# Tarekbouamer/Image-Retrieval-for-Image-Based-Localization

Measured on AMD Instinct MI355X. Metric: images/sec extract + queries/sec 1M-desc kNN, ResNet50-GeM 1024×768, higher is better.
Workload: dtype fp16

## Files before the change

image-retrieval-for-image-based-localization_amd/csrc/rr_c3pair.hip:

```cpp
#include "rr_internal.h"

#ifndef C3P_IG2
#define C3P_IG2 1
#endif

namespace rr {

namespace {

typedef __attribute__((ext_vector_type(4))) float cf32x4_t;
typedef __attribute__((ext_vector_type(4))) int ci32x4_t;

constexpr unsigned COOB = 0x80000000u;

__device__ __forceinline__ void cdma16(ci32x4_t rsrc, unsigned voff, unsigned lds_addr) {
    unsigned keep;
    lds_addr = __builtin_amdgcn_readfirstlane(lds_addr);
    asm volatile(
        "s_mov_b32 %0, m0\n\t"
        "s_mov_b32 m0, %3\n\t"
        "s_nop 0\n\t"
        "buffer_load_dwordx4 %1, %2, 0 offen lds\n\t"
        "s_mov_b32 m0, %0"
        : "=&s"(keep)
        : "v"(voff), "s"(rsrc), "s"(lds_addr)
        : "memory");
}

__device__ __forceinline__ ci32x4_t crsrc(const void* base, unsigned bytes) {
    const unsigned long long b = (unsigned long long)base;
    ci32x4_t r;
    r.x = __builtin_amdgcn_readfirstlane((int)(unsigned)b);
    r.y = __builtin_amdgcn_readfirstlane((int)((unsigned)(b >> 32) & 0xFFFFu));
    r.z = __builtin_amdgcn_readfirstlane((int)bytes);
    r.w = 0x00020000;
    int x = r.x, y = r.y, z = r.z;
    asm volatile("s_nop 4" : "+s"(x), "+s"(y), "+s"(z));
    r.x = x;
    r.y = y;
    r.z = z;
    return r;
}

__device__ __forceinline__ void cbar() { asm volatile("s_waitcnt lgkmcnt(0)\n\ts_barrier" ::: "memory"); }

template <int K>
__device__ __forceinline__ int cwswz(int row, int chunk) {
    const int f = K == 64 ? ((row >> 1) & 7) : (row & 15);
    return row * (K * 2) + ((chunk ^ f) << 4);
}

__device__ __forceinline__ void cpin(uint4& v) { asm volatile("" : "+v"(v.x), "+v"(v.y), "+v"(v.z), "+v"(v.w)); }

}

struct C3PairArgs {
    const bf16_t* t1;
    const bf16_t* w0;
    const float *s0, *h0;
    const bf16_t* w33;
    const float *s33, *h33;
    const bf16_t* w3;
    const float *s3, *h3;
    const bf16_t* res;
    const bf16_t* xp;
    const bf16_t* wp;
    const float *sp, *hp;
    const bf16_t* w1;
    const float *s1, *h1;
    bf16_t* y;
    bf16_t* z;
    int* queue;
    int n, h, w;
    int act2, act3, act1, act0;
    float slope2, slope3, slope1, slope0;
};

namespace {

template <int C1, bool PROJ, typename HT, bool CONV1 = false>
__global__ void __launch_bounds__(512, 1) k_c3pair(C3PairArgs a, int tiles_w, int tiles_hw, int ntiles) {
    static_assert(!CONV1 || PROJ, "conv1 in the launch: the stage's first block only");
    constexpr int TH = 4, TW = 32, TP = TH * TW, PITCH = 40;
    constexpr int NSLOT = (TH + 2) * PITCH, NP = NSLOT / 8;
    constexpr int PCW = TW + 2;
    constexpr int FN = 4;
    constexpr int K3 = 64, C3 = 256, NK3 = K3 / 32, NR3 = C3 / 32, NF1 = C1 / 16, NK1 = C3 / 32;
    static_assert(NSLOT % 8 == 0 && PITCH % 8 == 0, "row-invariant patch swizzle");
    __shared__ __attribute__((aligned(1024))) char sPatch[NSLOT * 128];
    __shared__ __attribute__((aligned(16))) char sT2[TP * 128];
    __shared__ __attribute__((aligned(16))) char sW3[C3 * K3 * 2];
    __shared__ __attribute__((aligned(16))) char sW1[C1 * C3 * 2];
    __shared__ __attribute__((aligned(16))) char sWp[PROJ ? C3 * K3 * 2 : 16];
    __shared__ __attribute__((aligned(16))) float sS3[C3], sH3[C3], sS1[C1], sH1[C1], sS2[64], sH2[64];
    __shared__ __attribute__((aligned(16))) float sSp[PROJ ? C3 : 4], sHp[PROJ ? C3 : 4];
    __shared__ __attribute__((aligned(16))) char sW0[CONV1 ? 64 * 64 * 2 : 16];
    __shared__ __attribute__((aligned(16))) float sS0[CONV1 ? 64 : 4], sH0[CONV1 ? 64 : 4];
    __shared__ int sTile[4];

    const int tid = threadIdx.x, lane = tid & 63;
    const int wave = __builtin_amdgcn_readfirstlane(tid >> 6);
    const bool role3 = wave < 4;
    const int r16 = lane & 15, kq = lane >> 4, lrow = lane >> 3, lch = lane & 7;
    const int H = a.h, W = a.w;

    for (int i = tid; i < C3 * K3 / 8; i += 512) {
        const int r = i / (K3 / 8), c = i - r * (K3 / 8);
        *reinterpret_cast<uint4*>(sW3 + cwswz<K3>(r, c)) = reinterpret_cast<const uint4*>(a.w3)[i];
        if constexpr (PROJ) *reinterpret_cast<uint4*>(sWp + cwswz<K3>(r, c)) = reinterpret_cast<const uint4*>(a.wp)[i];
    }
    for (int i = tid; i < C1 * C3 / 8; i += 512) {
        const int r = i / (C3 / 8), c = i - r * (C3 / 8);
        *reinterpret_cast<uint4*>(sW1 + cwswz<C3>(r, c)) = reinterpret_cast<const uint4*>(a.w1)[i];
    }
    for (int i = tid; i < C3; i += 512) {
        sS3[i] = a.s3[i];
        sH3[i] = a.h3[i];
        if constexpr (PROJ) {
            sSp[i] = a.sp[i];
            sHp[i] = a.hp[i];
        }
    }
    for (int i = tid; i < C1; i += 512) {
        sS1[i] = a.s1[i];
        sH1[i] = a.h1[i];
    }
    if (tid < 64) {
        sS2[tid] = a.s33[tid];
        sH2[tid] = a.h33[tid];
        if constexpr (CONV1) {
            sS0[tid] = a.s0[tid];
            sH0[tid] = a.h0[tid];
        }
    }
    if constexpr (CONV1)
        for (int i = tid; i < 64 * 64 / 8; i += 512) {
            const int r = i / 8, c = i - r * 8;
            *reinterpret_cast<uint4*>(sW0 + cwswz<64>(r, c)) = reinterpret_cast<const uint4*>(a.w0)[i];
        }
    const int wc = wave & 1, wpx = (wave >> 1) & 1;

    const int b = (int)blockIdx.x, G = (int)gridDim.x, xcd = b & 7;
    const int nt8 = ntiles >> 3, rt8 = ntiles & 7;
    const int s_x = xcd < rt8 ? xcd * (nt8 + 1) : rt8 * (nt8 + 1) + (xcd - rt8) * nt8;
    const int n_x = nt8 + (xcd < rt8 ? 1 : 0);
    auto fetch_tile = [&](int i) __attribute__((always_inline)) {
        if (a.queue) {
            const int v = atomicAdd(a.queue + xcd, 1);
            return v < n_x ? s_x + v : -1;
        }
        const int t = i * G + xcd * (G >> 3) + (b >> 3);
        return t < ntiles ? t : -1;
    };
    if (tid == 0) {
        sTile[0] = fetch_tile(0);
        sTile[1] = fetch_tile(1);
        sTile[2] = fetch_tile(2);
    }
    __syncthreads();
    auto tile_id = [&](int i) __attribute__((always_inline)) { return sTile[i & 3]; };
    if (tile_id(0) < 0) return;
    auto tile_org = [&](int t, int& img, int& oh0, int& ow0) __attribute__((always_inline)) {
        img = t / tiles_hw;
        const int rem = t - img * tiles_hw, th = rem / tiles_w;
        oh0 = th * TH;
        ow0 = (rem - th * tiles_w) * TW;
    };

    const ci32x4_t rsX = crsrc(a.t1, (unsigned)((long long)a.n * H * W * 64 * 2));
    const unsigned ldsP = (unsigned)(unsigned long long)sPatch;
    auto patch_dma = [&](int t, bool live) __attribute__((always_inline)) {
        int img = 0, oh0 = 0, ow0 = 0;
        if (live) tile_org(t, img, oh0, ow0);
        int lr = lrow;
        asm volatile("" : "+v"(lr));
#pragma unroll
        for (int u = 0; u < 8; ++u) {
            const int d = wave + 4 * u, q = d * 8 + lr;
            if (d >= NP) break;
            const int pr = q / PITCH, pc = q - pr * PITCH;
            const int hh = oh0 - 1 + pr, ww = ow0 - 1 + pc;
            unsigned off = COOB;
            if (live && pc < PCW && (unsigned)hh < (unsigned)H && (unsigned)ww < (unsigned)W)
                off = (unsigned)(((((long long)img * H + hh) * W + ww) * 64 + ((lch ^ lr) << 3)) * 2);
            cdma16(rsX, off, ldsP + d * 1024);
        }
    };
    h16_f32x4_t acc[2][FN];
    auto conv3x3 = [&](const uint4 (&areg)[2][18]) __attribute__((always_inline)) {
        int lc;
        asm volatile("v_mbcnt_lo_u32_b32 %0, -1, 0\n\tv_mbcnt_hi_u32_b32 %0, -1, %0" : "=v"(lc));
        lc &= 15;
        const char* base[FN][3][2];
#pragma unroll
        for (int j = 0; j < FN; ++j)
#pragma unroll
            for (int dx = 0; dx < 3; ++dx)
#pragma unroll
                for (int hs = 0; hs < 2; ++hs) {
                    const int q = (wpx * 2 + (j >> 1)) * PITCH + (j & 1) * 16 + lc + dx;
                    base[j][dx][hs] = sPatch + q * 128 + (((kq + 4 * hs) ^ (q & 7)) << 4);
                }
#pragma unroll
        for (int ii = 0; ii < 2; ++ii)
#pragma unroll
            for (int j = 0; j < FN; ++j) acc[ii][j] = (h16_f32x4_t){0.f, 0.f, 0.f, 0.f};
#pragma unroll
        for (int s = 0; s < 18; ++s) {
            const int tap = s >> 1, hs = s & 1, dy = tap / 3, dx = tap % 3;
            uint4 fb[FN];
#pragma unroll
            for (int j = 0; j < FN; ++j) fb[j] = *reinterpret_cast<const uint4*>(base[j][dx][hs] + dy * PITCH * 128);
#pragma unroll
            for (int ii = 0; ii < 2; ++ii)
#pragma unroll
                for (int j = 0; j < FN; ++j) acc[ii][j] = H16<HT>::mfma(areg[ii][s], fb[j], acc[ii][j]);
        }
    };
    auto convert_patch = [&](int t) __attribute__((always_inline)) {
        if constexpr (CONV1) {
            int img, oh0, ow0;
            tile_org(t, img, oh0, ow0);
            const bool leaky0 = a.act0 == RR_ACT_LEAKY;
            for (int f = wave; f < NP * 8 / 16; f += 4) {
                int q = f * 16 + r16;
                asm volatile("" : "+v"(q));
                const int pr = q / PITCH, pc = q - pr * PITCH;
                const int hh = oh0 - 1 + pr, ww = ow0 - 1 + pc;
                const bool valid = pc < PCW && (unsigned)hh < (unsigned)H && (unsigned)ww < (unsigned)W;
                char* slot = sPatch + q * 128;
                uint4 bx[2];
#pragma unroll
                for (int kk = 0; kk < 2; ++kk)
                    bx[kk] = *reinterpret_cast<const uint4*>(slot + (((4 * kk + kq) ^ (q & 7)) << 4));
                h16_f32x4_t c0[4];
#pragma unroll
                for (int ii = 0; ii < 4; ++ii) c0[ii] = (h16_f32x4_t){0.f, 0.f, 0.f, 0.f};
#pragma unroll
                for (int kk = 0; kk < 2; ++kk)
#pragma unroll
                    for (int ii = 0; ii < 4; ++ii) {
                        const uint4 av = *reinterpret_cast<const uint4*>(sW0 + cwswz<64>(ii * 16 + r16, kk * 4 + kq));
                        c0[ii] = H16<HT>::mfma(av, bx[kk], c0[ii]);
                    }
#pragma unroll
                for (int i2 = 0; i2 < 2; ++i2) {
                    const int c = 32 * i2 + 8 * kq;
                    float v[8];
#pragma unroll
                    for (int r = 0; r < 4; ++r) {
                        v[r] = c0[2 * i2][r] * sS0[c + r] + sH0[c + r];
                        v[4 + r] = c0[2 * i2 + 1][r] * sS0[c + 4 + r] + sH0[c + 4 + r];
                    }
                    if (leaky0) {
#pragma unroll
                        for (int r = 0; r < 8; ++r) v[r] = v[r] > 0.f ? v[r] : v[r] * a.slope0;
                    }
                    uint4 o = make_uint4(0u, 0u, 0u, 0u);
                    if (valid) {
                        o.x = H16<HT>::pack2(v[0], v[1]);
                        o.y = H16<HT>::pack2(v[2], v[3]);
                        o.z = H16<HT>::pack2(v[4], v[5]);
                        o.w = H16<HT>::pack2(v[6], v[7]);
                    }
                    *reinterpret_cast<uint4*>(slot + (((4 * i2 + kq) ^ (q & 7)) << 4)) = o;
                }
            }
        }
    };
    auto store_t2 = [&]() __attribute__((always_inline)) {
        const int c = 32 * wc + 8 * kq;
        float sc[8], sh[8];
#pragma unroll
        for (int r = 0; r < 8; ++r) {
            sc[r] = sS2[c + r];
            sh[r] = sH2[c + r];
        }
        const bool leaky2 = a.act2 == RR_ACT_LEAKY;
#pragma unroll
        for (int j = 0; j < FN; ++j) {
            const int p = wpx * (TP / 2) + j * 16 + r16;
            float v[8];
#pragma unroll
            for (int r = 0; r < 4; ++r) {
                v[r] = acc[0][j][r] * sc[r] + sh[r];
                v[4 + r] = acc[1][j][r] * sc[4 + r] + sh[4 + r];
            }
            if (leaky2) {
#pragma unroll
                for (int r = 0; r < 8; ++r) v[r] = v[r] > 0.f ? v[r] : v[r] * a.slope2;
            }
            uint4 o;
            o.x = H16<HT>::pack2(v[0], v[1]);
            o.y = H16<HT>::pack2(v[2], v[3]);
            o.z = H16<HT>::pack2(v[4], v[5]);
            o.w = H16<HT>::pack2(v[6], v[7]);
            *reinterpret_cast<uint4*>(sT2 + p * 128 + (((4 * wc + kq) ^ (p & 7)) << 4)) = o;
        }
    };

    const int pw = wave - 4;
    const bool leaky3 = a.act3 == RR_ACT_LEAKY, leaky1 = a.act1 == RR_ACT_LEAKY;
    constexpr int NRQ = PROJ ? NK3 : NR3;
    auto strip_pixel = [&](int t, int k) __attribute__((always_inline)) {
        int img, oh0, ow0;
        tile_org(t, img, oh0, ow0);
        return ((long long)img * H + oh0 + (k >> 1)) * W + ow0 + (k & 1) * 16 + r16;
    };
    auto load_rq = [&](uint4 (&dst)[NRQ], long long p) __attribute__((always_inline)) {
        if constexpr (PROJ) {
            const bf16_t* ps = a.xp + p * K3 + 8 * kq;
#pragma unroll
            for (int kk = 0; kk < NK3; ++kk) dst[kk] = ld16_once(ps + kk * 32);
        } else {
            const bf16_t* rs = a.res + p * C3 + 8 * kq;
#pragma unroll
            for (int i2 = 0; i2 < NR3; ++i2) dst[i2] = ld16_once(rs + 32 * i2);
        }
    };
    auto pair_strip = [&](int k, long long p, const uint4 (&rv)[NRQ]) __attribute__((always_inline)) {
        uint4 bq[NK3];
        {
            const int q = k * 16 + r16;
#pragma unroll
            for (int kk = 0; kk < NK3; ++kk)
                bq[kk] = *reinterpret_cast<const uint4*>(sT2 + q * 128 + (((4 * kk + kq) ^ (q & 7)) << 4));
        }
        uint4 yq[NR3];
        constexpr int IG = C3P_IG2 ? 2 : 1;
#pragma unroll
        for (int i0 = 0; i0 < NR3; i0 += IG) {
            int abase = 0;
            asm volatile("" : "+v"(abase));
            h16_f32x4_t acc3[IG][2], pacc[IG][2];
#pragma unroll
            for (int g = 0; g < IG; ++g)
#pragma unroll
                for (int hh = 0; hh < 2; ++hh) acc3[g][hh] = pacc[g][hh] = (h16_f32x4_t){0.f, 0.f, 0.f, 0.f};
#pragma unroll
            for (int kk = 0; kk < NK3; ++kk)
#pragma unroll
                for (int g = 0; g < IG; ++g)
#pragma unroll
                    for (int hh = 0; hh < 2; ++hh) {
                        const uint4 av = *reinterpret_cast<const uint4*>(sW3 + abase + cwswz<K3>((2 * (i0 + g) + hh) * 16 + r16, kk * 4 + kq));
                        acc3[g][hh] = H16<HT>::mfma(av, bq[kk], acc3[g][hh]);
                    }
            if constexpr (PROJ) {
#pragma unroll
                for (int kk = 0; kk < NK3; ++kk)
#pragma unroll
                    for (int g = 0; g < IG; ++g)
#pragma unroll
                        for (int hh = 0; hh < 2; ++hh) {
                            const uint4 av = *reinterpret_cast<const uint4*>(sWp + abase + cwswz<K3>((2 * (i0 + g) + hh) * 16 + r16, kk * 4 + kq));
                            pacc[g][hh] = H16<HT>::mfma(av, rv[kk], pacc[g][hh]);
                        }
            }
#pragma unroll
            for (int g = 0; g < IG; ++g) {
                const int i2 = i0 + g;
                const int c = 32 * i2 + 8 * kq;
                float v[8];
#pragma unroll
                for (int r = 0; r < 4; ++r) {
                    v[r] = acc3[g][0][r] * sS3[c + r] + sH3[c + r];
                    v[4 + r] = acc3[g][1][r] * sS3[c + 4 + r] + sH3[c + 4 + r];
                }
                if constexpr (PROJ) {
#pragma unroll
                    for (int r = 0; r < 4; ++r) {
                        v[r] += pacc[g][0][r] * sSp[c + r] + sHp[c + r];
                        v[4 + r] += pacc[g][1][r] * sSp[c + 4 + r] + sHp[c + 4 + r];
                    }
                } else {
                    const uint4 qv = rv[i2];
                    const unsigned w4[4] = {qv.x, qv.y, qv.z, qv.w};
#pragma unroll
                    for (int r = 0; r < 4; ++r) {
                        v[2 * r] += H16<HT>::lo(w4[r]);
                        v[2 * r + 1] += H16<HT>::hi(w4[r]);
                    }
                }
                if (leaky3) {
#pragma unroll
                    for (int r = 0; r < 8; ++r) v[r] = v[r] > 0.f ? v[r] : v[r] * a.slope3;
                }
                yq[i2].x = H16<HT>::pack2(v[0], v[1]);
                yq[i2].y = H16<HT>::pack2(v[2], v[3]);
                yq[i2].z = H16<HT>::pack2(v[4], v[5]);
                yq[i2].w = H16<HT>::pack2(v[6], v[7]);
                st16_once(a.y + p * C3 + c, yq[i2]);
            }
        }
        h16_f32x4_t zacc[NF1];
#pragma unroll
        for (int o = 0; o < NF1; ++o) zacc[o] = (h16_f32x4_t){0.f, 0.f, 0.f, 0.f};
#pragma unroll
        for (int kk = 0; kk < NK1; ++kk) {
            int abase = 0;
            asm volatile("" : "+v"(abase));
#pragma unroll
            for (int o = 0; o < NF1; ++o) {
                const uint4 av = *reinterpret_cast<const uint4*>(sW1 + abase + cwswz<C3>(o * 16 + r16, kk * 4 + kq));
                zacc[o] = H16<HT>::mfma(av, yq[kk], zacc[o]);
            }
        }
#pragma unroll
        for (int o2 = 0; o2 < NF1 / 2; ++o2) {
            const int c = 32 * o2 + 8 * kq;
            float v[8];
#pragma unroll
            for (int r = 0; r < 4; ++r) {
                v[r] = zacc[2 * o2][r] * sS1[c + r] + sH1[c + r];
                v[4 + r] = zacc[2 * o2 + 1][r] * sS1[c + 4 + r] + sH1[c + 4 + r];
            }
            if (leaky1) {
#pragma unroll
                for (int r = 0; r < 8; ++r) v[r] = v[r] > 0.f ? v[r] : v[r] * a.slope1;
            }
            uint4 o;
            o.x = H16<HT>::pack2(v[0], v[1]);
            o.y = H16<HT>::pack2(v[2], v[3]);
            o.z = H16<HT>::pack2(v[4], v[5]);
            o.w = H16<HT>::pack2(v[6], v[7]);
            st16_once(a.z + p * C1 + c, o);
        }
    };

    if (role3) {
        uint4 areg[2][18];
#pragma unroll
        for (int i = 0; i < 2; ++i)
#pragma unroll
            for (int ks = 0; ks < 18; ++ks)
                areg[i][ks] = *reinterpret_cast<const uint4*>(a.w33 + (long long)(32 * wc + 16 * i + r16) * 576 +
                                                              (ks >> 1) * 64 + 32 * (ks & 1) + 8 * kq);
#pragma unroll
        for (int i = 0; i < 2; ++i)
#pragma unroll
            for (int ks = 0; ks < 18; ++ks) cpin(areg[i][ks]);
        auto conv = [&]() __attribute__((always_inline)) { conv3x3(areg); };
        patch_dma(tile_id(0), true);
        asm volatile("s_waitcnt vmcnt(0)" ::: "memory");
        cbar();
        if constexpr (CONV1) {
            convert_patch(tile_id(0));
            cbar();
        }
        conv();
        if (wpx == 0) store_t2();
        cbar();
        patch_dma(tile_id(1), tile_id(1) >= 0);
        asm volatile("s_waitcnt vmcnt(0)" ::: "memory");
        cbar();
        for (int s = 0; tile_id(s) >= 0; ++s) {
            const bool more = tile_id(s + 1) >= 0;
            if (wpx == 1) store_t2();
            if constexpr (CONV1) {
                if (more) convert_patch(tile_id(s + 1));
                cbar();
            }
            if (more) conv();
            cbar();
            if (more) {
                if (wpx == 0) store_t2();
                const int t2i = tile_id(s + 2);
                patch_dma(t2i, t2i >= 0);
                if (tid == 0) sTile[(s + 3) & 3] = t2i >= 0 ? fetch_tile(s + 3) : -1;
                asm volatile("s_waitcnt vmcnt(0)" ::: "memory");
            }
            cbar();
        }
    } else {
        __builtin_amdgcn_s_setprio(1);
        uint4 rq[4][NRQ];
        load_rq(rq[0], strip_pixel(tile_id(0), pw));
        load_rq(rq[1], strip_pixel(tile_id(0), 4 + pw));
        cbar();
        if constexpr (CONV1) cbar();
        cbar();
        cbar();
        for (int s = 0; tile_id(s) >= 0; s += 2) {
            {
                const int t = tile_id(s);
                const bool n1 = tile_id(s + 1) >= 0;
                if (n1) load_rq(rq[2], strip_pixel(tile_id(s + 1), pw));
                if constexpr (CONV1) cbar();
                pair_strip(pw, strip_pixel(t, pw), rq[0]);
                cbar();
                if (n1) load_rq(rq[3], strip_pixel(tile_id(s + 1), 4 + pw));
                pair_strip(4 + pw, strip_pixel(t, 4 + pw), rq[1]);
                cbar();
            }
            if (tile_id(s + 1) >= 0) {
                const int t = tile_id(s + 1);
                const bool n2 = tile_id(s + 2) >= 0;
                if (n2) load_rq(rq[0], strip_pixel(tile_id(s + 2), pw));
                if constexpr (CONV1) cbar();
                pair_strip(pw, strip_pixel(t, pw), rq[2]);
                cbar();
                if (n2) load_rq(rq[1], strip_pixel(tile_id(s + 2), 4 + pw));
                pair_strip(4 + pw, strip_pixel(t, 4 + pw), rq[3]);
                cbar();
            }
        }
    }
}

}

}

using namespace rr;

extern "C" int rr_conv3x3_pair(const void* t1, int n, int h, int w, const void* w0, const float* scale0,
                               const float* shift0, int act0, float slope0, const void* w33, const float* scale2,
                               const float* shift2, int act2, float slope2, const void* w3, const float* scale3,
                               const float* shift3, const void* residual, const void* xp, const void* wp,
                               const float* scalep, const float* shiftp, int act3, float slope3, const void* w1,
                               const float* scale1, const float* shift1, int c_out, int act1, float slope1, void* y,
                               void* z, int* tile_queue, int dtype, void* stream) {
    if (dtype != RR_BF16 && dtype != RR_F16) return fail(RR_EINVAL, "rr_conv3x3_pair: dtype (bf16 / fp16)");
    if (!t1 || !w33 || !scale2 || !shift2 || !w3 || !scale3 || !shift3 || !w1 || !scale1 || !shift1 || !y || !z)
        return fail(RR_EINVAL, "rr_conv3x3_pair: null pointer");
    const bool proj = residual == nullptr;
    if (proj && (!xp || !wp || !scalep || !shiftp))
        return fail(RR_EINVAL, "rr_conv3x3_pair: either residual or the projection (xp, wp, scalep, shiftp)");
    if (c_out != 64 && c_out != 128) return fail(RR_EINVAL, "rr_conv3x3_pair: c_out 64 or 128");
    if (proj && c_out != 64) return fail(RR_EINVAL, "rr_conv3x3_pair: the projection form takes c_out = 64");
    const bool conv1 = w0 != nullptr;
    if (conv1 && (!proj || !scale0 || !shift0 || ((uintptr_t)w0 & 15)))
        return fail(RR_EINVAL, "rr_conv3x3_pair: conv1 in the launch (w0) needs the projection form, scale0, shift0");
    if (conv1 && act0 != RR_ACT_IDENTITY && act0 != RR_ACT_LEAKY) return fail(RR_EINVAL, "rr_conv3x3_pair: act0");
    if (n <= 0 || h <= 0 || w <= 0 || h % 4 || w % 32) return fail(RR_EINVAL, "rr_conv3x3_pair: h % 4, w % 32");
    if ((long long)n * h * w * 64 * 2 >= (1ll << 31)) return fail(RR_EINVAL, "rr_conv3x3_pair: t1 over 2 GiB (split the batch)");
    for (const void* p : {t1, w33, w3, residual, xp, wp, w1, (const void*)y, (const void*)z})
        if ((uintptr_t)p & 15) return fail(RR_EINVAL, "rr_conv3x3_pair: 16-byte alignment required");
    if ((uintptr_t)tile_queue & 3) return fail(RR_EINVAL, "rr_conv3x3_pair: tile_queue alignment");
    for (int act : {act2, act3, act1})
        if (act != RR_ACT_IDENTITY && act != RR_ACT_LEAKY) return fail(RR_EINVAL, "rr_conv3x3_pair: activation");
    C3PairArgs a;
    a.t1 = (const bf16_t*)t1; a.w33 = (const bf16_t*)w33; a.s33 = scale2; a.h33 = shift2;
    a.w3 = (const bf16_t*)w3; a.s3 = scale3; a.h3 = shift3; a.res = (const bf16_t*)residual;
    a.xp = (const bf16_t*)xp; a.wp = (const bf16_t*)wp; a.sp = scalep; a.hp = shiftp;
    a.w1 = (const bf16_t*)w1; a.s1 = scale1; a.h1 = shift1; a.y = (bf16_t*)y; a.z = (bf16_t*)z;
    a.n = n; a.h = h; a.w = w; a.act2 = act2; a.act3 = act3; a.act1 = act1;
    a.slope2 = slope2; a.slope3 = slope3; a.slope1 = slope1; a.queue = tile_queue;
    a.w0 = (const bf16_t*)w0; a.s0 = scale0; a.h0 = shift0; a.act0 = act0; a.slope0 = slope0;
    const int tiles_w = w / 32, tiles_hw = (h / 4) * tiles_w;
    const long long ntl = (long long)n * tiles_hw;
    if (ntl >= (1ll << 31)) return fail(RR_EINVAL, "rr_conv3x3_pair: too many tiles");
    const int cus = grid_cus();
    int grid = (int)(ntl < cus ? ntl : cus) & ~7;
    if (grid < 8) grid = 8;
    const dim3 g((unsigned)grid), b(512);
    hipStream_t s = as_stream(stream);
    auto go = [&](auto hv) {
        using H = decltype(hv);
        if (conv1) hipLaunchKernelGGL((k_c3pair<64, true, H, true>), g, b, 0, s, a, tiles_w, tiles_hw, (int)ntl);
        else if (proj) hipLaunchKernelGGL((k_c3pair<64, true, H>), g, b, 0, s, a, tiles_w, tiles_hw, (int)ntl);
        else if (c_out == 64) hipLaunchKernelGGL((k_c3pair<64, false, H>), g, b, 0, s, a, tiles_w, tiles_hw, (int)ntl);
        else hipLaunchKernelGGL((k_c3pair<128, false, H>), g, b, 0, s, a, tiles_w, tiles_hw, (int)ntl);
    };
    if (dtype == RR_F16) go(f16_t{});
    else go(bf16_t{});
    return check_launch("rr_conv3x3_pair");
}
```

image-retrieval-for-image-based-localization_amd/csrc/rr_stream.hip:

```cpp
#include "rr_internal.h"

namespace rr {

namespace {

typedef __attribute__((ext_vector_type(4))) float sf32x4_t;

template <int K>
__device__ __forceinline__ int wswz(int row, int chunk) {
    const int f = K == 64 ? ((row >> 1) & 7) : (row & 15);
    return row * (K * 2) + ((chunk ^ f) << 4);
}

template <int TC, int K, int FN, int D, int NW, bool RES, typename H>
__global__ void __launch_bounds__(64 * NW) k_stream1x1(ConvArgs a, int nslices, int xmap) {
    constexpr int NI = TC / 16;
    constexpr int NK = K / 32;
    constexpr int NR = TC / 32;
    constexpr int SP = 16 * FN;
    constexpr bool AREG = NI * NK * 4 <= 32;
    __shared__ __attribute__((aligned(16))) char sA[TC * K * 2];
    __shared__ __attribute__((aligned(16))) float sS[TC], sH[TC];

    const int tid = threadIdx.x, lane = tid & 63;
// ... 741 lines not shown
template <int K, int CW, bool RES, typename H, bool DEEP = true>
__global__ void __launch_bounds__(512, 1) k_wres1x1(WresArgs a) {
    constexpr int TP = 32, NJ = TP / 16, NI = CW / 16, NK = K / 32, BC = 8 * CW;
    constexpr int XRB = K * 2, RRB = RES ? BC * 2 : 0;
    constexpr int XB = TP * XRB, RB = TP * RRB;
    constexpr int BUF = XB + RB, NBUF = RES || !DEEP ? 3 : (BUF <= 16384 ? 6 : 4), DA = NBUF - 1;
    constexpr int NDX = XB / 1024 / 8, NDR = RB / 1024 / 8;
    constexpr int ND = NDX + NDR, NST = (CW / 32) * NJ;
    static_assert(NI * NK <= 32 && XB % 8192 == 0 && RB % 8192 == 0, "tile shape");
    static_assert(XRB <= 1024 && RRB <= 1024, "row fits one DMA instruction");
    __shared__ __attribute__((aligned(1024))) char smem[NBUF * BUF];
    __shared__ __attribute__((aligned(16))) float sS[BC], sH[BC];

    const int tid = threadIdx.x, lane = tid & 63;
    const int wave = __builtin_amdgcn_readfirstlane(tid >> 6);
    const int r16 = lane & 15, kq = lane >> 4;
    const int b = (int)blockIdx.x, ns = a.nslices;
    const int slice = a.xmap ? (b >> 3) % ns : b % ns;
    const int bi = a.xmap ? ((b >> 3) / ns) * 8 + (b & 7) : b / ns;
    const int G = (int)gridDim.x / ns;
    const int c0 = slice * BC, cw0 = c0 + CW * wave;

    const bool affine = a.scale != nullptr;
    for (int i = tid; i < BC; i += 512) {
        sS[i] = affine ? a.scale[c0 + i] : 1.f;
        sH[i] = affine ? a.shift[c0 + i] : 0.f;
    }
    uint4 areg[NI][NK];
#pragma unroll
    for (int i = 0; i < NI; ++i)
#pragma unroll
        for (int kk = 0; kk < NK; ++kk)
            areg[i][kk] = *reinterpret_cast<const uint4*>(a.w + (long long)(cw0 + 16 * i + r16) * K + 32 * kk + 8 * kq);
#pragma unroll
    for (int i = 0; i < NI; ++i)
#pragma unroll
        for (int kk = 0; kk < NK; ++kk) pin_loaded(areg[i][kk]);
    __syncthreads();

    const long long P = a.P;
    const int ntiles = (int)((P + TP - 1) / TP);
    if (bi >= ntiles) return;
    const long long nimg = P / ((long long)a.ho * a.wo);
    const si32x4_t rsX = srsrc(a.x, (unsigned)(nimg * a.h * a.w_ * XRB));
    si32x4_t rsR = rsX;
    if constexpr (RES) rsR = srsrc(a.res + c0, (unsigned)(P * a.ldy * 2 - (long long)c0 * 2));
    const unsigned lds0 = (unsigned)(unsigned long long)smem;
    const int hw = a.ho * a.wo;
    auto x_row = [&](unsigned p) -> unsigned {
        if (a.stride == 1) return p;
        const unsigned img = p / (unsigned)hw, rem = p - img * (unsigned)hw;
        const unsigned oh = rem / (unsigned)a.wo, ow = rem - oh * (unsigned)a.wo;
        return (img * (unsigned)a.h + oh * (unsigned)a.stride) * (unsigned)a.w_ + ow * (unsigned)a.stride;
    };
    auto dma = [&](int t, int buf) {
#pragma unroll
        for (int u = 0; u < NDX; ++u) {
            constexpr int CPR = XRB / 16;
            const int d = NDX * wave + u, px = d * (1024 / XRB) + lane / CPR, slot = lane % CPR;
            const unsigned off = x_row((unsigned)(t * TP + px)) * XRB + (unsigned)((slot ^ (px & 15)) << 4);
            sdma16(rsX, off, lds0 + buf * BUF + d * 1024);
        }
        if constexpr (RES) {
#pragma unroll
            for (int u = 0; u < NDR; ++u) {
                constexpr int CPR = RRB / 16;
                const int d = NDR * wave + u, px = d * (1024 / RRB) + lane / CPR, slot = lane % CPR;
                const unsigned off = (unsigned)(((long long)t * TP + px) * a.ldy * 2) + (unsigned)((slot ^ (px & 15)) << 4);
                sdma16(rsR, off, lds0 + buf * BUF + XB + d * 1024);
            }
        }
    };
    const bool leaky = a.act == RR_ACT_LEAKY;

    if constexpr (DA == 2) {
        dma(bi, 0);
        if (bi + G < ntiles) dma(bi + G, 1);
    } else {
#pragma unroll
        for (int j = 0; j < DA; ++j) dma(bi + j * G, j);
    }
    for (int k = 0, t = bi; t < ntiles; ++k, t += G) {
        const int cur = k % NBUF;
        if constexpr (DA == 2) {
            if (t + G < ntiles) {
                if (k == 0) asm volatile("s_waitcnt vmcnt(%0)\n\ts_barrier" ::"n"(ND) : "memory");
                else asm volatile("s_waitcnt vmcnt(%0)\n\ts_barrier" ::"n"(ND + NST) : "memory");
            } else {
                if (k == 0) asm volatile("s_waitcnt vmcnt(0)\n\ts_barrier" ::: "memory");
                else asm volatile("s_waitcnt vmcnt(%0)\n\ts_barrier" ::"n"(NST) : "memory");
            }
            if (t + 2 * G < ntiles) dma(t + 2 * G, (k + 2) % NBUF);
        } else {
            if (k == 0) asm volatile("s_waitcnt vmcnt(%0)\n\ts_barrier" ::"n"((DA - 1) * ND) : "memory");
            else asm volatile("s_waitcnt vmcnt(%0)\n\ts_barrier" ::"n"((DA - 1) * ND + NST) : "memory");
            dma(t + DA * G, (k + DA) % NBUF);
        }
        const char* X = smem + cur * BUF;
        const char* Rt = X + XB;
        h16_f32x4_t acc[NI][NJ];
#pragma unroll
        for (int i = 0; i < NI; ++i)
#pragma unroll
            for (int j = 0; j < NJ; ++j) acc[i][j] = (h16_f32x4_t){0.f, 0.f, 0.f, 0.f};
#pragma unroll
        for (int kk = 0; kk < NK; ++kk) {
            uint4 bx[NJ];
#pragma unroll
            for (int j = 0; j < NJ; ++j) {
                const int px = 16 * j + r16;
                bx[j] = *reinterpret_cast<const uint4*>(X + px * XRB + (((4 * kk + kq) ^ (px & 15)) << 4));
            }
#pragma unroll
            for (int i = 0; i < NI; ++i)
#pragma unroll
                for (int j = 0; j < NJ; ++j) acc[i][j] = H16<H>::mfma(areg[i][kk], bx[j], acc[i][j]);
        }
#pragma unroll
        for (int i2 = 0; i2 < CW / 32; ++i2) {
            const int cl = CW * wave + 32 * i2 + 8 * kq;
            const float4 sc0 = *reinterpret_cast<const float4*>(sS + cl);
            const float4 sc1 = *reinterpret_cast<const float4*>(sS + cl + 4);
            const float4 sh0 = *reinterpret_cast<const float4*>(sH + cl);
            const float4 sh1 = *reinterpret_cast<const float4*>(sH + cl + 4);
            const float sc[8] = {sc0.x, sc0.y, sc0.z, sc0.w, sc1.x, sc1.y, sc1.z, sc1.w};
            const float sh[8] = {sh0.x, sh0.y, sh0.z, sh0.w, sh1.x, sh1.y, sh1.z, sh1.w};
#pragma unroll
            for (int j = 0; j < NJ; ++j) {
                const int px = 16 * j + r16;
                float v[8];
#pragma unroll
                for (int r = 0; r < 4; ++r) {
                    v[r] = acc[2 * i2][j][r] * sc[r] + sh[r];
                    v[4 + r] = acc[2 * i2 + 1][j][r] * sc[4 + r] + sh[4 + r];
                }
                if constexpr (RES) {
                    const uint4 q = *reinterpret_cast<const uint4*>(Rt + px * RRB + (((cl >> 3) ^ (px & 15)) << 4));
                    const unsigned w4[4] = {q.x, q.y, q.z, q.w};
#pragma unroll
                    for (int r = 0; r < 4; ++r) {
                        v[2 * r] += H16<H>::lo(w4[r]);
                        v[2 * r + 1] += H16<H>::hi(w4[r]);
                    }
                }
                if (leaky) {
#pragma unroll
                    for (int r = 0; r < 8; ++r) v[r] = v[r] > 0.f ? v[r] : v[r] * a.slope;
                }
                uint4 o;
                o.x = H16<H>::pack2(v[0], v[1]);
                o.y = H16<H>::pack2(v[2], v[3]);
                o.z = H16<H>::pack2(v[4], v[5]);
                o.w = H16<H>::pack2(v[6], v[7]);
                const long long p = (long long)t * TP + px;
                if (p < P) st16_once(a.y + p * a.ldy + c0 + cl, o);
            }
        }
    }
    asm volatile("s_waitcnt vmcnt(0)" ::: "memory");
}


template <int TC, int K, int FN, int D, int NW, typename H>
void launch_s_t(const ConvArgs& a, hipStream_t s) {
    const int g_stream_cus = grid_cus();
    constexpr int LDS = TC * K * 2 + TC * 8;
    constexpr int PER_CU = (160 * 1024 / LDS) >= 2 && NW <= 8 ? (NW <= 4 ? 4 : 2) : 1;
    const int nslices = a.cout / TC;
    const long long nstrips = ((long long)a.P + 16 * FN - 1) / (16 * FN);
    long long per_slice = (long long)PER_CU * g_stream_cus / nslices;
    if (per_slice < 1) per_slice = 1;
    const long long need = (nstrips + NW - 1) / NW;
    if (per_slice > need) per_slice = need;
    const int grid = (int)(per_slice * nslices);
    const int xmap = g_tune.stream_xcd && nslices > 1 && grid % (8 * nslices) == 0;
    if (a.flags & RR_CONV_RESIDUAL)
        hipLaunchKernelGGL((k_stream1x1<TC, K, FN, D, NW, true, H>), dim3(grid), dim3(64 * NW), 0, s, a, nslices, xmap);
    else
        hipLaunchKernelGGL((k_stream1x1<TC, K, FN, D, NW, false, H>), dim3(grid), dim3(64 * NW), 0, s, a, nslices, xmap);
}

template <int K, int CW>
void launch_wres(const ConvArgs& a, hipStream_t s, bool f16) {
    constexpr int BC = 8 * CW;
    const bool res = a.flags & RR_CONV_RESIDUAL;
    WresArgs w;
    w.w = (const bf16_t*)a.w;
    const bool affine = a.flags & RR_CONV_AFFINE;
    w.scale = affine ? a.scale : nullptr;
    w.shift = affine ? a.shift : nullptr;
    w.ldy = a.ldy;
    w.act = a.act;
    w.slope = a.slope;
    w.h = a.h; w.w_ = a.w_; w.ho = a.ho; w.wo = a.wo; w.stride = a.stride;
    w.nslices = a.cout / BC;
    int per = grid_cus() / w.nslices;
    if (per < 1) per = 1;
    const long long in_img = (long long)a.h * a.w_ * K * 2, out_img = (long long)a.ho * a.wo * a.ldy * 2;
    long long ich = (1ll << 31) / (in_img > out_img ? in_img : out_img);
    if (ich < 1) ich = 1;
    const long long hw = (long long)a.ho * a.wo;
    for (long long i0 = 0; i0 < a.n; i0 += ich) {
        const long long ni = a.n - i0 < ich ? a.n - i0 : ich;
        w.x = (const bf16_t*)a.x + i0 * a.h * a.w_ * K;
        w.res = res ? (const bf16_t*)a.res + i0 * hw * a.ldy : nullptr;
        w.y = (bf16_t*)a.y + i0 * hw * a.ldy;
        w.P = ni * hw;
        const long long ntiles = (w.P + 31) / 32;
        const int ps = (int)(per < ntiles ? per : ntiles);
        const int grid = ps * w.nslices;
        w.xmap = w.nslices > 1 && grid % (8 * w.nslices) == 0;
        auto go = [&](auto h) {
            using H = decltype(h);
            if (res) hipLaunchKernelGGL((k_wres1x1<K, CW, true, H>), dim3(grid), dim3(512), 0, s, w);
            else if (g_tune.wres_ring) hipLaunchKernelGGL((k_wres1x1<K, CW, false, H>), dim3(grid), dim3(512), 0, s, w);
            else hipLaunchKernelGGL((k_wres1x1<K, CW, false, H, false>), dim3(grid), dim3(512), 0, s, w);
        };
        if (f16) go(f16_t{});
        else go(bf16_t{});
    }
}
}

template <int TC, int K, int FN, int D, int NW>
void launch_s(const ConvArgs& a, hipStream_t s, bool f16) {
    if (f16) launch_s_t<TC, K, FN, D, NW, f16_t>(a, s);
    else launch_s_t<TC, K, FN, D, NW, bf16_t>(a, s);
}

bool gemm8_eligible(const ConvArgs& a, bool k1, int esz);

bool launch_stream1x1(const ConvArgs& a, hipStream_t s, bool f16) {
    if (g_tune.stream_1x1 == 0) return false;
    if (!(a.flags & RR_CONV_PERM32) || a.kh != 1 || a.kw != 1 || a.pad != 0 || a.kp != a.cin) return false;
    if (a.P < 4096 || (long long)a.n * a.h * a.w_ * a.cin >= (1ll << 31)) return false;
    const bool res = a.flags & RR_CONV_RESIDUAL;
    const int K = a.cin, C = a.cout;
    if (g_tune.wres && (a.ldy & 7) == 0 && (a.stride == 1 ? a.h == a.ho && a.w_ == a.wo : !res)) {
        if (K == 512 && C == 2048 && res) { launch_wres<512, 32>(a, s, f16); return true; }
        if (K == 256 && C == 1024 && res) { launch_wres<256, 64>(a, s, f16); return true; }
        if (K == 128 && C == 512 && res) { launch_wres<128, 64>(a, s, f16); return true; }
        if (g_tune.wres >= 2) {
            if (K == 512 && (C == 256 || C == 1024 || C == 2048) && !res) { launch_wres<512, 32>(a, s, f16); return true; }
            if (K == 256 && (C == 512 || C == 1024) && !res) { launch_wres<256, 64>(a, s, f16); return true; }
        }
    }
    if (g_tune.stream_1x1 >= 2 && K == 512 && C == 2048 && res && gemm8_eligible(a, true, 2)) return false;
    if (g_tune.stream_1x1 >= 3 && K == 256 && C == 1024 && res && gemm8_eligible(a, true, 2)) return false;
    if (K == 64 && C == 64) { launch_s<64, 64, 2, 4, 8>(a, s, f16); return true; }
    if (K == 64 && C == 256) { launch_s<256, 64, 1, 2, 8>(a, s, f16); return true; }
    if (K == 256 && C == 64) { launch_s<64, 256, 1, 4, 8>(a, s, f16); return true; }
    if (K == 256 && C == 128) { launch_s<128, 256, 1, 3, 8>(a, s, f16); return true; }
    if (K == 128 && C == 512) { launch_s<256, 128, 1, 3, 8>(a, s, f16); return true; }
    if (K == 512 && C == 128) { launch_s<128, 512, 1, 2, 8>(a, s, f16); return true; }
    if (K == 256 && C == 1024 && res) { launch_s<256, 256, 1, 2, 8>(a, s, f16); return true; }
    if (K == 256 && C == 512 && !res) { launch_s<256, 256, 1, 2, 8>(a, s, f16); return true; }
    if (K == 512 && C == 2048 && res) { launch_s<128, 512, 1, 2, 8>(a, s, f16); return true; }
    if (K == 512 && !res && (C == 256 || C == 1024) && gemm8_eligible(a, true, 2)) return false;
    if (K == 512 && C == 256 && !res) { launch_s<128, 512, 1, 2, 8>(a, s, f16); return true; }
    if (K == 512 && C == 1024 && !res) { launch_s<128, 512, 1, 2, 8>(a, s, f16); return true; }
    return false;
}


}

using namespace rr;

extern "C" int rr_conv1x1_pair(const void* x, long long p, int c_in, const void* w3, const float* scale3,
                               const float* shift3, int c_mid, const void* residual, const void* xp, const void* wp,
                               const float* scalep, const float* shiftp, int act3, float slope3, const void* w1,
                               const float* scale1, const float* shift1, int c_out, int act1, float slope1, void* y,
                               void* z, int dtype, void* stream) {
    if (dtype != RR_BF16 && dtype != RR_F16) return fail(RR_EINVAL, "rr_conv1x1_pair: bf16 / fp16 only");
    const bool stage2 = c_in == 64 && c_mid == 256 && (c_out == 64 || c_out == 128);
    const bool stage3 = c_in == 128 && c_mid == 512 && c_out == 128;
    if (!stage2 && !stage3)
        return fail(RR_EINVAL, "rr_conv1x1_pair: shapes (c_in 64, c_mid 256, c_out 64|128) or (128, 512, 128) only");
    if (!x || !w3 || !scale3 || !shift3 || !w1 || !scale1 || !shift1 || !y || !z)
        return fail(RR_EINVAL, "rr_conv1x1_pair: null pointer");
    const bool proj = residual == nullptr;
    if (proj && stage3) return fail(RR_EINVAL, "rr_conv1x1_pair: the 128/512 boundary needs a residual");
    if (proj && (!xp || !wp || !scalep || !shiftp))
        return fail(RR_EINVAL, "rr_conv1x1_pair: either residual or the projection (xp, wp, scalep, shiftp) is required");
    if (proj && ((((uintptr_t)xp) | ((uintptr_t)wp)) & 15))
        return fail(RR_EINVAL, "rr_conv1x1_pair: 16-byte alignment required");
    if (p <= 0) return fail(RR_EINVAL, "rr_conv1x1_pair: empty");
    if ((((uintptr_t)x) | ((uintptr_t)residual) | ((uintptr_t)y) | ((uintptr_t)z) | ((uintptr_t)w3) |
         ((uintptr_t)w1)) & 15)
        return fail(RR_EINVAL, "rr_conv1x1_pair: 16-byte alignment required");
    if (act3 != RR_ACT_IDENTITY && act3 != RR_ACT_LEAKY) return fail(RR_EINVAL, "rr_conv1x1_pair: act3");
    if (act1 != RR_ACT_IDENTITY && act1 != RR_ACT_LEAKY) return fail(RR_EINVAL, "rr_conv1x1_pair: act1");
    const int g_pair_cus = grid_cus();
    hipStream_t s = as_stream(stream);
    if (stage3) {
        constexpr long long CH = 1ll << 20;
        for (long long p0 = 0; p0 < p; p0 += CH) {
            PairMidArgs m;
            const long long pn = p - p0 < CH ? p - p0 : CH;
            m.x = (const bf16_t*)x + p0 * 128; m.w3 = (const bf16_t*)w3; m.s3 = scale3; m.h3 = shift3;
            m.res = (const bf16_t*)residual + p0 * 512; m.w1 = (const bf16_t*)w1; m.s1 = scale1; m.h1 = shift1;
            m.y = (bf16_t*)y + p0 * 512; m.z = (bf16_t*)z + p0 * 128; m.P = pn;
            m.act3 = act3; m.act1 = act1; m.slope3 = slope3; m.slope1 = slope1;
            const long long ntiles = (pn + (g_tune.pair_mid ? 31 : 63)) / (g_tune.pair_mid ? 32 : 64);
            const int grid = (int)(ntiles < g_pair_cus ? ntiles : g_pair_cus);
            if (g_tune.pair_mid) {
                if (dtype == RR_F16) hipLaunchKernelGGL(k_pair_mid_ring<f16_t>, dim3(grid), dim3(512), 0, s, m);
                else hipLaunchKernelGGL(k_pair_mid_ring<bf16_t>, dim3(grid), dim3(512), 0, s, m);
            } else {
                if (dtype == RR_F16) hipLaunchKernelGGL(k_pair_mid<f16_t>, dim3(grid), dim3(512), 0, s, m);
                else hipLaunchKernelGGL(k_pair_mid<bf16_t>, dim3(grid), dim3(512), 0, s, m);
            }
        }
        return check_launch("rr_conv1x1_pair");
    }
    PairArgs a;
    a.x = (const bf16_t*)x; a.w3 = (const bf16_t*)w3; a.s3 = scale3; a.h3 = shift3; a.res = (const bf16_t*)residual;
    a.w1 = (const bf16_t*)w1; a.s1 = scale1; a.h1 = shift1; a.y = (bf16_t*)y; a.z = (bf16_t*)z; a.P = p;
    a.act3 = act3; a.act1 = act1; a.slope3 = slope3; a.slope1 = slope1;
    a.xp = (const bf16_t*)xp; a.wp = (const bf16_t*)wp; a.sp = scalep; a.hp = shiftp;
    const long long nstrips = (p + 15) / 16;
    long long grid = (nstrips + 7) / 8;
    if (grid > g_pair_cus) grid = g_pair_cus;
    const dim3 g((unsigned)grid), b(512);
    auto go = [&](auto h) {
        using H = decltype(h);
        if (c_out == 64 && !proj) hipLaunchKernelGGL((k_stream_pair<64, 2, false, H>), g, b, 0, s, a);
        else if (c_out == 64) hipLaunchKernelGGL((k_stream_pair<64, 2, true, H>), g, b, 0, s, a);
        else if (!proj) hipLaunchKernelGGL((k_stream_pair<128, 2, false, H>), g, b, 0, s, a);
        else hipLaunchKernelGGL((k_stream_pair<128, 2, true, H>), g, b, 0, s, a);
    };
    if (dtype == RR_F16) go(f16_t{});
    else go(bf16_t{});
    return check_launch("rr_conv1x1_pair");
}
```

Baseline: 5658.

## Keep projection-block 1x1 weights in VGPRs and DMA projection input via LDS

Adds a VP variant of the fused 3x3+1x1 pair kernel for the projection block, used by default. The 1x1 pair role now holds conv3, projection and conv1 weights in registers instead of LDS. The projection input is DMA'd into LDS in half tiles alongside the patch prefetch, and the two 1x1 stages are software-pipelined across half tiles through an LDS staging buffer for y. The aim is to remove LDS weight reads and overlap the stages, at the cost of much higher register pressure and extra LDS for the x and y buffers. The pair_mid tune flag is split into bits so the ring and VP paths can each be toggled.

```diff
diff --git a/image-retrieval-for-image-based-localization_amd/csrc/rr_c3pair.hip b/image-retrieval-for-image-based-localization_amd/csrc/rr_c3pair.hip
--- a/image-retrieval-for-image-based-localization_amd/csrc/rr_c3pair.hip
+++ b/image-retrieval-for-image-based-localization_amd/csrc/rr_c3pair.hip
@@ -78,9 +78,10 @@
 
 namespace {
 
-template <int C1, bool PROJ, typename HT, bool CONV1 = false>
+template <int C1, bool PROJ, typename HT, bool CONV1 = false, bool VP = false>
 __global__ void __launch_bounds__(512, 1) k_c3pair(C3PairArgs a, int tiles_w, int tiles_hw, int ntiles) {
     static_assert(!CONV1 || PROJ, "conv1 in the launch: the stage's first block only");
+    static_assert(!VP || (PROJ && !CONV1 && C1 == 64), "weights-in-VGPRs pair role: the projection form");
     constexpr int TH = 4, TW = 32, TP = TH * TW, PITCH = 40;
     constexpr int NSLOT = (TH + 2) * PITCH, NP = NSLOT / 8;
     constexpr int PCW = TW + 2;
@@ -89,9 +90,12 @@
     static_assert(NSLOT % 8 == 0 && PITCH % 8 == 0, "row-invariant patch swizzle");
     __shared__ __attribute__((aligned(1024))) char sPatch[NSLOT * 128];
     __shared__ __attribute__((aligned(16))) char sT2[TP * 128];
-    __shared__ __attribute__((aligned(16))) char sW3[C3 * K3 * 2];
-    __shared__ __attribute__((aligned(16))) char sW1[C1 * C3 * 2];
-    __shared__ __attribute__((aligned(16))) char sWp[PROJ ? C3 * K3 * 2 : 16];
+    __shared__ __attribute__((aligned(16))) char sW3[VP ? 16 : C3 * K3 * 2];
+    __shared__ __attribute__((aligned(16))) char sW1[VP ? 16 : C1 * C3 * 2];
+    __shared__ __attribute__((aligned(16))) char sWp[PROJ && !VP ? C3 * K3 * 2 : 16];
+    constexpr int PP = TP / 2, YB = PP * C3 * 2, XB = PP * K3 * 2;
+    __shared__ __attribute__((aligned(1024))) char sX[VP ? 2 * XB : 16];
+    __shared__ __attribute__((aligned(16))) char sY[VP ? 2 * YB : 16];
     __shared__ __attribute__((aligned(16))) float sS3[C3], sH3[C3], sS1[C1], sH1[C1], sS2[64], sH2[64];
     __shared__ __attribute__((aligned(16))) float sSp[PROJ ? C3 : 4], sHp[PROJ ? C3 : 4];
     __shared__ __attribute__((aligned(16))) char sW0[CONV1 ? 64 * 64 * 2 : 16];
@@ -104,14 +108,16 @@
     const int r16 = lane & 15, kq = lane >> 4, lrow = lane >> 3, lch = lane & 7;
     const int H = a.h, W = a.w;
 
-    for (int i = tid; i < C3 * K3 / 8; i += 512) {
-        const int r = i / (K3 / 8), c = i - r * (K3 / 8);
-        *reinterpret_cast<uint4*>(sW3 + cwswz<K3>(r, c)) = reinterpret_cast<const uint4*>(a.w3)[i];
-        if constexpr (PROJ) *reinterpret_cast<uint4*>(sWp + cwswz<K3>(r, c)) = reinterpret_cast<const uint4*>(a.wp)[i];
-    }
-    for (int i = tid; i < C1 * C3 / 8; i += 512) {
-        const int r = i / (C3 / 8), c = i - r * (C3 / 8);
-        *reinterpret_cast<uint4*>(sW1 + cwswz<C3>(r, c)) = reinterpret_cast<const uint4*>(a.w1)[i];
+    if constexpr (!VP) {
+        for (int i = tid; i < C3 * K3 / 8; i += 512) {
+            const int r = i / (K3 / 8), c = i - r * (K3 / 8);
+            *reinterpret_cast<uint4*>(sW3 + cwswz<K3>(r, c)) = reinterpret_cast<const uint4*>(a.w3)[i];
+            if constexpr (PROJ) *reinterpret_cast<uint4*>(sWp + cwswz<K3>(r, c)) = reinterpret_cast<const uint4*>(a.wp)[i];
+        }
+        for (int i = tid; i < C1 * C3 / 8; i += 512) {
+            const int r = i / (C3 / 8), c = i - r * (C3 / 8);
+            *reinterpret_cast<uint4*>(sW1 + cwswz<C3>(r, c)) = reinterpret_cast<const uint4*>(a.w1)[i];
+        }
     }
     for (int i = tid; i < C3; i += 512) {
         sS3[i] = a.s3[i];
@@ -186,6 +192,22 @@
             cdma16(rsX, off, ldsP + d * 1024);
         }
     };
+    ci32x4_t rsXp = rsX;
+    if constexpr (VP) rsXp = crsrc(a.xp, (unsigned)((long long)a.n * H * W * 64 * 2));
+    const unsigned ldsX = (unsigned)(unsigned long long)sX;
+    auto x_dma = [&](int t, int half) __attribute__((always_inline)) {
+        int img, oh0, ow0;
+        tile_org(t, img, oh0, ow0);
+        int lr = lrow;
+        asm volatile("" : "+v"(lr));
+#pragma unroll
+        for (int u = 0; u < 2; ++u) {
+            const int d = wave + 4 * u, q = d * 8 + lr;
+            const int hh = oh0 + 2 * half + (q >> 5), ww = ow0 + (q & 31);
+            const unsigned off = (unsigned)(((((long long)img * H + hh) * W + ww) * 64 + ((lch ^ lr) << 3)) * 2);
+            cdma16(rsXp, off, ldsX + half * XB + d * 1024);
+        }
+    };
     h16_f32x4_t acc[2][FN];
     auto conv3x3 = [&](const uint4 (&areg)[2][18]) __attribute__((always_inline)) {
         int lc;
@@ -452,6 +474,7 @@
         if (wpx == 0) store_t2();
         cbar();
         patch_dma(tile_id(1), tile_id(1) >= 0);
+        if constexpr (VP) x_dma(tile_id(0), 0);
         asm volatile("s_waitcnt vmcnt(0)" ::: "memory");
         cbar();
         for (int s = 0; tile_id(s) >= 0; ++s) {
@@ -461,17 +484,170 @@
                 if (more) convert_patch(tile_id(s + 1));
                 cbar();
             }
+            if constexpr (VP) x_dma(tile_id(s), 1);
             if (more) conv();
+            if constexpr (VP) asm volatile("s_waitcnt vmcnt(0)" ::: "memory");
             cbar();
             if (more) {
                 if (wpx == 0) store_t2();
                 const int t2i = tile_id(s + 2);
                 patch_dma(t2i, t2i >= 0);
+                if constexpr (VP) x_dma(tile_id(s + 1), 0);
                 if (tid == 0) sTile[(s + 3) & 3] = t2i >= 0 ? fetch_tile(s + 3) : -1;
                 asm volatile("s_waitcnt vmcnt(0)" ::: "memory");
             }
             cbar();
         }
+    } else if constexpr (VP) {
+        __builtin_amdgcn_s_setprio(1);
+        const int rh = pw & 1, sh = pw >> 1;
+        const float slope3e = leaky3 ? a.slope3 : 1.f, slope1e = leaky1 ? a.slope1 : 1.f;
+        uint4 a3[4][NK3], ap[4][NK3], a1[2][NK1];
+#pragma unroll
+        for (int f = 0; f < 4; ++f)
+#pragma unroll
+            for (int kk = 0; kk < NK3; ++kk) {
+                const long long o = (long long)((4 * pw + f) * 16 + r16) * K3 + kk * 32 + 8 * kq;
+                a3[f][kk] = *reinterpret_cast<const uint4*>(a.w3 + o);
+                ap[f][kk] = *reinterpret_cast<const uint4*>(a.wp + o);
+            }
+#pragma unroll
+        for (int hh = 0; hh < 2; ++hh)
+#pragma unroll
+            for (int kk = 0; kk < NK1; ++kk)
+                a1[hh][kk] = *reinterpret_cast<const uint4*>(a.w1 + (long long)((2 * rh + hh) * 16 + r16) * C3 + kk * 32 + 8 * kq);
+#pragma unroll
+        for (int f = 0; f < 4; ++f)
+#pragma unroll
+            for (int kk = 0; kk < NK3; ++kk) {
+                cpin(a3[f][kk]);
+                cpin(ap[f][kk]);
+            }
+#pragma unroll
+        for (int hh = 0; hh < 2; ++hh)
+#pragma unroll
+            for (int kk = 0; kk < NK1; ++kk) cpin(a1[hh][kk]);
+        auto half_pixel = [&](int t, int half) __attribute__((always_inline)) {
+            int img, oh0, ow0;
+            tile_org(t, img, oh0, ow0);
+            return ((long long)img * H + oh0 + 2 * half) * W + ow0 + r16;
+        };
+        auto stage1 = [&](int t, int half) __attribute__((always_inline)) {
+            const long long p0 = half_pixel(t, half);
+            int ln = lane;
+            asm volatile("" : "+v"(ln));
+            const int r16 = ln & 15, kq = ln >> 4;
+#pragma unroll
+            for (int k = 0; k < 4; ++k) {
+                const int q = k * 16 + r16;
+                const long long p = p0 + (long long)(k >> 1) * W + (k & 1) * 16;
+                int kqa = kq;
+                asm volatile("" : "+v"(kqa));
+                uint4 bq[NK3], xq[NK3];
+#pragma unroll
+                for (int kk = 0; kk < NK3; ++kk) {
+                    const int o = q * 128 + (((4 * kk + kq) ^ (q & 7)) << 4);
+                    bq[kk] = *reinterpret_cast<const uint4*>(sT2 + half * (PP * 128) + o);
+                    xq[kk] = *reinterpret_cast<const uint4*>(sX + half * XB + o);
+                }
+                h16_f32x4_t acc3[2][2], pacc[2][2];
+#pragma unroll
+                for (int g = 0; g < 2; ++g)
+#pragma unroll
+                    for (int hh = 0; hh < 2; ++hh) acc3[g][hh] = pacc[g][hh] = (h16_f32x4_t){0.f, 0.f, 0.f, 0.f};
+#pragma unroll
+                for (int kk = 0; kk < NK3; ++kk)
+#pragma unroll
+                    for (int g = 0; g < 2; ++g)
+#pragma unroll
+                        for (int hh = 0; hh < 2; ++hh) acc3[g][hh] = H16<HT>::mfma(a3[2 * g + hh][kk], bq[kk], acc3[g][hh]);
+#pragma unroll
+                for (int kk = 0; kk < NK3; ++kk)
+#pragma unroll
+                    for (int g = 0; g < 2; ++g)
+#pragma unroll
+                        for (int hh = 0; hh < 2; ++hh) pacc[g][hh] = H16<HT>::mfma(ap[2 * g + hh][kk], xq[kk], pacc[g][hh]);
+#pragma unroll
+                for (int g = 0; g < 2; ++g) {
+                    const int i2 = 2 * pw + g;
+                    const int c = 32 * i2 + 8 * kqa;
+                    float v[8];
+#pragma unroll
+                    for (int r = 0; r < 4; ++r) {
+                        v[r] = acc3[g][0][r] * sS3[c + r] + sH3[c + r];
+                        v[4 + r] = acc3[g][1][r] * sS3[c + 4 + r] + sH3[c + 4 + r];
+                    }
+#pragma unroll
+                    for (int r = 0; r < 4; ++r) {
+                        v[r] += pacc[g][0][r] * sSp[c + r] + sHp[c + r];
+                        v[4 + r] += pacc[g][1][r] * sSp[c + 4 + r] + sHp[c + 4 + r];
+                    }
+#pragma unroll
+                    for (int r = 0; r < 8; ++r) v[r] = v[r] > 0.f ? v[r] : v[r] * slope3e;
+                    uint4 o;
+                    o.x = H16<HT>::pack2(v[0], v[1]);
+                    o.y = H16<HT>::pack2(v[2], v[3]);
+                    o.z = H16<HT>::pack2(v[4], v[5]);
+                    o.w = H16<HT>::pack2(v[6], v[7]);
+                    st16_once(a.y + p * C3 + c, o);
+                    *reinterpret_cast<uint4*>(sY + half * YB + q * (C3 * 2) + (((4 * i2 + kq) ^ (q & 15)) << 4)) = o;
+                }
+            }
+        };
+        auto stage2 = [&](int t, int half) __attribute__((always_inline)) {
+            const long long p0 = half_pixel(t, half);
+            int ln = lane;
+            asm volatile("" : "+v"(ln));
+            const int r16 = ln & 15, kq = ln >> 4;
+            h16_f32x4_t zacc[2][2];
+#pragma unroll
+            for (int ks = 0; ks < 2; ++ks)
+#pragma unroll
+                for (int hh = 0; hh < 2; ++hh) zacc[ks][hh] = (h16_f32x4_t){0.f, 0.f, 0.f, 0.f};
+#pragma unroll
+            for (int kk = 0; kk < NK1; ++kk)
+#pragma unroll
+                for (int ks = 0; ks < 2; ++ks) {
+                    const int q = (2 * sh + ks) * 16 + r16;
+                    const uint4 yv = *reinterpret_cast<const uint4*>(sY + half * YB + q * (C3 * 2) + (((4 * kk + kq) ^ (q & 15)) << 4));
+#pragma unroll
+                    for (int hh = 0; hh < 2; ++hh) zacc[ks][hh] = H16<HT>::mfma(a1[hh][kk], yv, zacc[ks][hh]);
+                }
+            const int c = 32 * rh + 8 * kq;
+#pragma unroll
+            for (int ks = 0; ks < 2; ++ks) {
+                const long long p = p0 + (long long)sh * W + ks * 16;
+                float v[8];
+#pragma unroll
+                for (int r = 0; r < 4; ++r) {
+                    v[r] = zacc[ks][0][r] * sS1[c + r] + sH1[c + r];
+                    v[4 + r] = zacc[ks][1][r] * sS1[c + 4 + r] + sH1[c + 4 + r];
+                }
+#pragma unroll
+                for (int r = 0; r < 8; ++r) v[r] = v[r] > 0.f ? v[r] : v[r] * slope1e;
+                uint4 o;
+                o.x = H16<HT>::pack2(v[0], v[1]);
+                o.y = H16<HT>::pack2(v[2], v[3]);
+                o.z = H16<HT>::pack2(v[4], v[5]);
+                o.w = H16<HT>::pack2(v[6], v[7]);
+                st16_once(a.z + p * C1 + c, o);
+            }
+        };
+        cbar();
+        cbar();
+        cbar();
+        int tp = -1;
+        for (int s = 0; tile_id(s) >= 0; ++s) {
+            const int t = tile_id(s);
+            stage1(t, 0);
+            if (tp >= 0) stage2(tp, 1);
+            cbar();
+            stage1(t, 1);
+            stage2(t, 0);
+            cbar();
+            tp = t;
+        }
+        stage2(tp, 1);
     } else {
         __builtin_amdgcn_s_setprio(1);
         uint4 rq[4][NRQ];
@@ -556,9 +732,11 @@
     if (grid < 8) grid = 8;
     const dim3 g((unsigned)grid), b(512);
     hipStream_t s = as_stream(stream);
+    const bool vp = !(g_tune.pair_mid & 2);
     auto go = [&](auto hv) {
         using H = decltype(hv);
         if (conv1) hipLaunchKernelGGL((k_c3pair<64, true, H, true>), g, b, 0, s, a, tiles_w, tiles_hw, (int)ntl);
+        else if (proj && vp) hipLaunchKernelGGL((k_c3pair<64, true, H, false, true>), g, b, 0, s, a, tiles_w, tiles_hw, (int)ntl);
         else if (proj) hipLaunchKernelGGL((k_c3pair<64, true, H>), g, b, 0, s, a, tiles_w, tiles_hw, (int)ntl);
         else if (c_out == 64) hipLaunchKernelGGL((k_c3pair<64, false, H>), g, b, 0, s, a, tiles_w, tiles_hw, (int)ntl);
         else hipLaunchKernelGGL((k_c3pair<128, false, H>), g, b, 0, s, a, tiles_w, tiles_hw, (int)ntl);
diff --git a/image-retrieval-for-image-based-localization_amd/csrc/rr_stream.hip b/image-retrieval-for-image-based-localization_amd/csrc/rr_stream.hip
--- a/image-retrieval-for-image-based-localization_amd/csrc/rr_stream.hip
+++ b/image-retrieval-for-image-based-localization_amd/csrc/rr_stream.hip
@@ -1067,9 +1067,10 @@
             m.res = (const bf16_t*)residual + p0 * 512; m.w1 = (const bf16_t*)w1; m.s1 = scale1; m.h1 = shift1;
             m.y = (bf16_t*)y + p0 * 512; m.z = (bf16_t*)z + p0 * 128; m.P = pn;
             m.act3 = act3; m.act1 = act1; m.slope3 = slope3; m.slope1 = slope1;
-            const long long ntiles = (pn + (g_tune.pair_mid ? 31 : 63)) / (g_tune.pair_mid ? 32 : 64);
+            const bool ring = g_tune.pair_mid & 1;
+            const long long ntiles = (pn + (ring ? 31 : 63)) / (ring ? 32 : 64);
             const int grid = (int)(ntiles < g_pair_cus ? ntiles : g_pair_cus);
-            if (g_tune.pair_mid) {
+            if (ring) {
                 if (dtype == RR_F16) hipLaunchKernelGGL(k_pair_mid_ring<f16_t>, dim3(grid), dim3(512), 0, s, m);
                 else hipLaunchKernelGGL(k_pair_mid_ring<bf16_t>, dim3(grid), dim3(512), 0, s, m);
             } else {
```

Result: no change. 5685 (median of 6 runs) (+0.5%).
